# MeteoSwiss/flexpart

Hardware: AMD Instinct MI355X
Metric: particle-steps/sec (whole node) + achieved HBM GB/s, 1e8 particles (higher is better)
Workload: dtype f64

## Files before the change

### flexpart_amd/_lib.py

```python
from __future__ import annotations

import ctypes as C
import os

HERE = os.path.dirname(os.path.abspath(__file__))
LIB_PATH = os.environ.get("FPX_LIBRARY") or os.path.join(HERE, "csrc", "libflexpart_amd.so")

FPX_MAXSPEC = 5
DEAD = -999999999
RNG_TABLE_SEQ, RNG_TABLE_COUNTER, RNG_PHILOX = 0, 1, 2


class FpxConfig(C.Structure):
    _fields_ = [
        ("struct_bytes", C.c_int32), ("device", C.c_int32),
        ("compute_real_bytes", C.c_int32), ("host_real_bytes", C.c_int32),
        ("max_particles", C.c_int64),
        ("nx", C.c_int32), ("ny", C.c_int32), ("nz", C.c_int32), ("nmixz", C.c_int32),
        ("nxmax", C.c_int32), ("nymax", C.c_int32), ("nzmax", C.c_int32),
        ("dx", C.c_double), ("dy", C.c_double), ("xlon0", C.c_double), ("ylat0", C.c_double),
        ("xglobal", C.c_int32), ("nglobal", C.c_int32), ("sglobal", C.c_int32),
        ("switchnorthg", C.c_double), ("switchsouthg", C.c_double),
        ("northpolemap", C.c_double * 9), ("southpolemap", C.c_double * 9),
        ("ldirect", C.c_int32), ("lsynctime", C.c_int32), ("method", C.c_int32),
# ... 131 lines not shown
class FpxStepStats(C.Structure):
    _fields_ = [(n, C.c_int64) for n in
                ("n_due", "n_initialized", "n_left_domain", "n_min_mass", "n_max_age",
                 "nan_count", "nan_count2", "n_bad_position")] + [("kernel_ms", C.c_double)]


ALLREDUCE_FN = C.CFUNCTYPE(C.c_int, C.c_void_p, C.c_void_p, C.c_void_p, C.c_int64, C.c_int32)

SYMBOLS = [
    "fpx_create", "fpx_destroy", "fpx_last_error", "fpx_abi_version", "fpx_polar_maps", "fpx_set_height",
    "fpx_upload_fields", "fpx_set_windtime", "fpx_rng_fill_table", "fpx_rng_set_table",
    "fpx_rng_get_table", "fpx_upload_particles", "fpx_download_particles", "fpx_set_numpart", "fpx_set_release_points", "fpx_set_release_heights", "fpx_release_init", "fpx_releaseparticles", "fpx_split_particles", "fpx_redist_plan", "fpx_redist_bytes", "fpx_redist_pack", "fpx_redist_unpack",
    "fpx_step", "fpx_step_async", "fpx_sync", "fpx_counters", "fpx_kernel_time", "fpx_kernel_times", "fpx_sort_particles",
    "fpx_seed_particles", "fpx_stream", "fpx_outgrid_init", "fpx_set_output_times", "fpx_conccalc",
    "fpx_get_grids", "fpx_comm_unique_id", "fpx_comm_init", "fpx_comm_init_host", "fpx_count_particles", "fpx_lane_stats", "fpx_set_option", "fpx_get_info", "fpx_wet_init", "fpx_upload_wet_fields",
    "fpx_wetdepo", "fpx_get_wetgrid", "fpx_nests_init", "fpx_upload_nest_fields", "fpx_math_probe",
    "fpx_outgrid_nest_init", "fpx_get_grids_nest", "fpx_receptors_init", "fpx_get_receptors", "fpx_upload_wet_nest_fields",
    "fpx_verttransform_ecmwf", "fpx_verttransform_nest", "fpx_verttransform_time", "fpx_calcpar", "fpx_calcpar_time", "fpx_upload_diag_fields", "fpx_partoutput", "fpx_partoutput_time", "fpx_readpartpositions", "fpx_concoutput",
    "fpx_checkpoint_write", "fpx_checkpoint_read",
    "fpx_conv_init", "fpx_upload_conv_fields", "fpx_convmix", "fpx_convmix_time", "fpx_get_cbaseflux", "fpx_set_cbaseflux",
    "fpx_upload_conv_nest_fields", "fpx_get_cbaseflux_nest", "fpx_set_cbaseflux_nest", "fpx_upload_diag_nest_fields",
]

_lib = None


def load():
    global _lib
    if _lib is not None:
        return _lib
    if not os.path.exists(LIB_PATH):
        raise ImportError(
            f"{LIB_PATH} not found: the HIP extension is not built "
            "(run `python -c 'import __graft_entry__ as g; g.build()'`). "
            "flexpart_amd has no CPU fallback.")
    lib = C.CDLL(LIB_PATH)
    vp = C.c_void_p
    lib.fpx_last_error.restype = C.c_char_p
    lib.fpx_stream.restype = vp
    lib.fpx_stream.argtypes = [vp]
    lib.fpx_math_probe.argtypes = [C.c_int32, vp, vp, C.c_int64]
    lib.fpx_upload_wet_nest_fields.argtypes = [vp, C.c_int32, C.c_int32, C.POINTER(FpxWetFields), C.c_int32]
    lib.fpx_outgrid_nest_init.argtypes = [vp, C.POINTER(FpxOutgridNest)]
    lib.fpx_get_grids_nest.argtypes = [vp, vp, vp, vp, C.c_int32, C.c_int32]
    lib.fpx_receptors_init.argtypes = [vp, C.c_int32, vp, vp, vp]
    lib.fpx_get_receptors.argtypes = [vp, vp, C.c_int32, C.c_int32, C.c_int32]
    lib.fpx_create.argtypes = [C.POINTER(vp), C.POINTER(FpxConfig)]
    lib.fpx_destroy.argtypes = [vp]
    lib.fpx_polar_maps.argtypes = [C.c_int32, C.c_double, C.POINTER(C.c_double), C.POINTER(C.c_double)]
    lib.fpx_set_height.argtypes = [vp, vp, C.c_int32]
    lib.fpx_upload_fields.argtypes = [vp, C.c_int32, C.POINTER(FpxFields)]
    lib.fpx_verttransform_ecmwf.argtypes = [vp, C.c_int32, C.POINTER(FpxModelLevels), C.POINTER(FpxFields), C.POINTER(FpxFieldsOut)]
    lib.fpx_verttransform_nest.argtypes = [vp, C.c_int32, C.c_int32, C.POINTER(FpxModelLevels), C.POINTER(FpxFields), C.POINTER(FpxFieldsOut)]
    lib.fpx_verttransform_time.argtypes = [vp, C.POINTER(C.c_double)]
    lib.fpx_calcpar.argtypes = [vp, C.c_int32, C.POINTER(FpxCalcparIn), C.POINTER(FpxCalcparOut)]
    lib.fpx_calcpar_time.argtypes = [vp, C.POINTER(C.c_double)]
# ... 75 lines not shown
```

### flexpart_amd/csrc/fpx_device.hpp

```cpp
#pragma once
#include "fpx_tu.hpp"
#include <hip/hip_runtime.h>
#include <stdint.h>

namespace fpx {
FPX_TU_OPEN

#define K(x) ((R)(x))
#define FPX_DEV __device__ __forceinline__
#define FPX_HD __host__ __device__ __forceinline__

constexpr int kMaxSpec = 5;
constexpr int kMaxNests = 4;
constexpr int kDead = -999999999;

FPX_HD float m_exp(float x) { return expf(x); }
FPX_HD double m_exp(double x) { return exp(x); }
FPX_HD float m_log(float x) { return logf(x); }
FPX_HD double m_log(double x) { return log(x); }
FPX_HD float m_sqrt(float x) { return sqrtf(x); }
FPX_HD double m_sqrt(double x) { return sqrt(x); }
FPX_HD float m_fma(float a, float b, float c) { return fmaf(a, b, c); }
FPX_HD double m_fma(double a, double b, double c) { return fma(a, b, c); }
FPX_HD float m_sin(float x) { return sinf(x); }
// ... 630 lines not shown
  const double r = m_rcbrt(x);
  const double d = ((1.0 / 3.0) - .33333) * M.logabs(x);
  return (x * (r * r)) * (1.0 - d * (1.0 - d * (0.5 - d * 0.16666666666666666)));
}
template <typename MS>
FPX_DEV float m_pow13(float x, const MS &) { return m_powr(x, 0.33333f); }

template <typename R, typename MS>
FPX_DEV R tlw_unstable(const Turb<R> &T, R z, const MS &M) {
  if (z < m_abs(T.ol)) return K(0.1) * z * m_rcp(T.sigw * (K(0.55) - K(0.38) * m_abs(z * m_rcp(T.ol))));
  if (T.zeta < K(0.1)) return K(0.59) * z * m_rcp(T.sigw);
  return K(0.15) * T.h * m_rcp(T.sigw) * (K(1.) - M.expt(K(-5) * T.zeta));
}

template <typename R, typename MS>
FPX_DEV void sigw_unstable(Turb<R> &T, const MS &M) {
  R z23, zm13;
  zeta_powers(T.zeta, M, z23, zm13);
  T.sigw = m_sqrtp(K(1.2) * (T.wst * T.wst) * (K(1.) - K(.9) * T.zeta) * z23 + (K(1.8) - K(1.4) * T.zeta) * (T.ust * T.ust)) + K(1.e-2);
  T.dsigwdz = K(0.5) * m_rcp(T.sigw * T.h) * (K(-1.4) * (T.ust * T.ust) + (T.wst * T.wst) * (K(0.8) * zm13 - K(1.8) * z23));
}

template <typename R, typename MS = PlainMath>
FPX_DEV void hanna(Turb<R> &T, R z, const MS &M = MS()) {
  if (T.h / m_abs(T.ol) < K(1.)) {
    T.ust = m_max(K(1.e-4), T.ust);
    R corr = z * m_rcp(T.ust);
    T.sigu = K(1.e-2) + K(2.0) * T.ust * M.expt(K(-3.e-4) * corr);
    T.sigw = K(1.3) * T.ust * M.expt(K(-2.e-4) * corr);
    T.dsigwdz = K(-2.e-4) * T.sigw;
    T.sigw = T.sigw + K(1.e-2);
    T.sigv = T.sigw;
    T.tlu = K(0.5) * z * m_rcp(T.sigw * (K(1.) + K(1.5e-3) * corr));
    T.tlv = T.tlu;
    T.tlw = T.tlu;
  } else if (T.ol < K(0.)) {
// ... 2 lines not shown
    sigw_unstable(T, M);
    T.tlu = K(0.15) * T.h * m_rcp(T.sigu);
    T.tlv = T.tlu;
    T.tlw = tlw_unstable(T, z, M);
  } else {
    T.sigu = K(1.e-2) + K(2.) * T.ust * (K(1.) - T.zeta);
    T.sigv = K(1.e-2) + K(1.3) * T.ust * (K(1.) - T.zeta);
    T.sigw = T.sigv;
    T.dsigwdz = K(-1.3) * T.ust * m_rcp(T.h);
    T.tlu = K(0.15) * T.h * m_rcp(T.sigu) * m_sqrtp(T.zeta);
    T.tlv = K(0.467) * T.tlu;
    T.tlw = K(0.1) * T.h * m_rcp(T.sigw) * m_pow08(T.zeta);
  }
  T.tlu = m_max(K(10.), T.tlu);
  T.tlv = m_max(K(10.), T.tlv);
  T.tlw = m_max(K(30.), T.tlw);
  if (T.dsigwdz == K(0.)) T.dsigwdz = K(1.e-10);
}

template <typename R>
FPX_DEV void hanna1(Turb<R> &T, R z) {
  if (T.h / m_abs(T.ol) < K(1.)) {
    T.ust = m_max(K(1.e-4), T.ust);
    T.sigu = K(2.0) * T.ust * m_exp(K(-3.e-4) * z / T.ust);
    T.sigu = m_max(T.sigu, K(1.e-5));
    T.sigv = K(1.3) * T.ust * m_exp(K(-2.e-4) * z / T.ust);
    T.sigv = m_max(T.sigv, K(1.e-5));
    T.sigw = T.sigv;
    T.dsigw2dz = K(-6.76e-4) * T.ust * m_exp(K(-4.e-4) * z / T.ust);
    T.tlu = K(0.5) * z / T.sigw / (K(1.) + K(1.5e-3) * z / T.ust);
// ... 36 lines not shown
    T.dsigw2dz = K(3.38) * T.ust * T.ust * (T.zeta - K(1.)) / T.h;
    T.tlu = K(0.15) * T.h / T.sigu * m_sqrt(T.zeta);
    T.tlv = K(0.467) * T.tlu;
    T.tlw = K(0.1) * T.h / T.sigw * m_powr(T.zeta, K(0.8));
  }
  T.tlu = m_max(K(10.), T.tlu);
  T.tlv = m_max(K(10.), T.tlv);
  T.tlw = m_max(K(30.), T.tlw);
}

enum StashSlot {
  S_U, S_V, S_W,
  S_DDX, S_DDY,
  S_DX, S_DY, S_DAW, S_DCW,
  S_UP, S_VP,
  S_UST, S_WST, S_OL, S_TRANS,
  S_RHOAUX,
  S_NPASS,
  S_COUNT_LEAN,
  S_TDEP = S_COUNT_LEAN,
  S_SETCELL,
  S_SET_NUM, S_SET_DQ6, S_SET_V0,
  S_COUNT_AERO64,
  S_RT_TAG = S_COUNT_AERO64, S_RT_RHO1, S_RT_TT1, S_RT_RHO2, S_RT_TT2,
  S_COUNT
};
template <typename R> constexpr int stash_slots(bool lean, bool susp = true) { return lean ? (susp ? (int)S_COUNT_LEAN : (int)S_NPASS) : (sizeof(R) == 8 ? (int)S_COUNT_AERO64 : (int)S_COUNT); }
constexpr int kStashStride = 256;
template <typename R>
struct Stash {
  typedef __attribute__((address_space(3))) volatile R *lds_ptr;
  lds_ptr p;
  lds_tab_ptr tab;
  FPX_DEV double logabs(double x) const { return m_log_abs(x, tab); }
  FPX_DEV double expt(double x) const { return m_exp_tab(x, tab + kLdsExpTabAt); }
  FPX_DEV float logabs(float x) const { return m_logp(x); }
  FPX_DEV float expt(float x) const { return m_expp(x); }
  FPX_DEV R get(int k) const { return p[k * kStashStride]; }
  FPX_DEV void put(int k, R v) const { p[k * kStashStride] = v; }
  FPX_DEV void add(int k, R v) const { p[k * kStashStride] = p[k * kStashStride] + v; }
};

template <typename R>
struct HsInv {
  R ih, iaux;
  int regime;
};
template <typename R>
FPX_DEV HsInv<R> hanna_short_prepare(Turb<R> &T) {
  HsInv<R> I;
  I.ih = m_rcp(T.h);
  if (T.h / m_abs(T.ol) < K(1.)) {
    I.regime = 0;
    T.ust = m_max(K(1.e-4), T.ust);
    I.iaux = m_rcp(T.ust);
  } else if (T.ol < K(0.)) {
    I.regime = 1;
    I.iaux = m_rcp(T.ol);
  } else {
    I.regime = 2;
    I.iaux = K(0.);
  }
  return I;
}

template <typename R, typename ST>
FPX_DEV void hanna_short(Turb<R> &T, R z, const HsInv<R> &I, const ST &S) {
  if (I.regime == 0) {
    const R corr = z * I.iaux;
    T.sigw = K(1.3) * S.expt(K(-2.e-4) * corr);
    T.dsigwdz = K(-2.e-4) * T.sigw;
    T.sigw = T.sigw * S.get(S_UST) + K(1.e-2);
    const R qn = K(1.) + K(1.5e-3) * corr;
    const R in2 = m_rcp(T.sigw * qn);
    T.isigw = in2 * qn;
    T.tlw = K(0.5) * z * in2;
  } else if (I.regime == 1) {
    R z23, zm13;
    zeta_powers(T.zeta, S, z23, zm13);
    const R ust = S.get(S_UST), wst = S.get(S_WST);
    const R ust2 = ust * ust, wst2 = wst * wst;
    T.sigw = m_sqrtp(K(1.2) * wst2 * (K(1.) - K(.9) * T.zeta) * z23 + (K(1.8) - K(1.4) * T.zeta) * ust2) + K(1.e-2);
    const bool low = z < m_abs(S.get(S_OL));
    const R q = low ? K(0.55) - K(0.38) * m_abs(z * I.iaux) : K(1.);
    const R i2 = m_rcp(T.sigw * q);
    const R isig = i2 * q;
    T.isigw = isig;
    T.dsigwdz = K(0.5) * isig * I.ih * (K(-1.4) * ust2 + wst2 * (K(0.8) * zm13 - K(1.8) * z23));
    if (low) T.tlw = K(0.1) * z * i2;
    else if (T.zeta < K(0.1)) T.tlw = K(0.59) * z * isig;
    else T.tlw = K(0.15) * T.h * isig * (K(1.) - S.expt(K(-5) * T.zeta));
  } else {
    const R ust = S.get(S_UST);
    T.sigw = K(1.e-2) + K(1.3) * ust * (K(1.) - T.zeta);
    T.dsigwdz = K(-1.3) * ust * I.ih;
    T.isigw = m_rcp(T.sigw);
// ... 10 lines not shown

template <typename R>
FPX_DEV R cuberoot(R x) { return m_sign(m_pow(m_abs(x), K(0.333333333)), x); }

template <typename R>
FPX_DEV R cbl_transition(R h, R ol) {
  R transition = K(1.);
  if (-h / ol < K(15)) transition = m_sin(((-h / ol + K(10.)) / K(10.)) * FPX_PI_PAR) / K(2.) + K(0.5);
  return transition;
}

template <typename R, typename ST>
FPX_DEV void cbl(const ST &S, int ldirect, R wp, R zp, R wt , R ih , R rhoaux , R sigmaw, R irw , R dsigmawdz, R tlw,
                 R &ath, R &bth, int &flagrein) {
  const R usurad2 = K(0.7071067812), usurad2p = K(0.3989422804), C0 = K(3), costluar4 = K(0.66667), eps = K(0.000001);
  const R timedir = (R)ldirect;
  const R z = zp * ih;
  const R w2 = sigmaw * sigmaw;
  const R rtl = m_rsqrt(tlw);
  const R alfa = (K(2.) / C0) * w2 * (rtl * rtl);
  const R wold = timedir * wp;
  const R omz = K(1.) - z;
  const R omz05 = m_sqrtp(omz), omz15 = omz * omz05;
  const R w3 = (K(1.2) * z * omz15 + eps) * wt;
  const R dw3 = (K(1.2) * (omz15 - z * K(1.5) * omz05)) * (wt * ih);
  const R irw2 = irw * irw, irw3 = irw2 * irw;
  const R skew = w3 * irw3;
  const R dskew = irw3 * dw3 - K(3.) * skew * dsigmawdz * irw;
  R fluarw = K(0.), dfluarw = K(0.), xluarw = K(0.), dxluarw = K(0.);
  if (skew != K(0)) {
    R croot, icroot2;
    m_cuberoot_parts(m_abs(skew), croot, icroot2);
    fluarw = costluar4 * m_sign(croot, skew);
    dfluarw = costluar4 * (K(1.) / K(3.)) * icroot2 * dskew;
  }
  const R fluarw2 = fluarw * fluarw;
// ... 37 lines not shown
  const R pb = (usurad2p * isb) * eb;
  const R aperfa = da * usurad2;
  const R aperfb = db * usurad2;
  const R rx = rhoaux;
  const R apa = aluarw * pa, bpb = bluarw * pb;
  const R ptot = apa + bpb;
  const R Ta = aluarw * (dwa + wa * rx) + wa * daluarw;
  const R Tb = bluarw * (dwb + wb * rx) + wb * dbluarw;
  const R wdf = wold * dfluarw;
  const R Ua = sigmawa * (aluarw * (dsigmawa * (wold2 * isa2 + K(1.)) + wdf) + sigmawa * (daluarw + rx * aluarw));
  const R Ub = sigmawb * (bluarw * (dsigmawb * (wold2 * isb2 + K(1.)) - wdf) + sigmawb * (dbluarw + rx * bluarw));
  const R cu = usurad2 * usurad2 - K(0.5);
  R erfa, erfb;
  m_erf_e2(aperfa, ea - ea * (da2 * cu), aperfb, eb - eb * (db2 * cu), erfa, erfb);
  const R Phi = K(0.5) * (Tb * erfb - Ta * erfa) + Ua * pa + Ub * pb;
  const R Q = timedir * ((da * isa) * apa + (db * isb) * bpb);
  ath = m_rcp(ptot) * (-(C0 / K(2.)) * alfa * Q + Phi);
  bth = (sigmaw * K(1.4142135623730951)) * rtl;
}

template <typename R>
FPX_DEV void cbl_pdf(R zp, R wst, R h, R sigmaw, R ol, R &aluarw, R &sigmawa, R &sigmawb, R &wa, R &wb) {
  const R costluar4 = K(0.66667), eps = K(0.000001);
  R z = zp / h;
  R transition = cbl_transition(h, ol);
  R w2 = sigmaw * sigmaw;
  const R omz = K(1.) - z;
  R w3 = ((K(1.2) * z * (omz * m_sqrt(omz)) + eps) * (wst * wst * wst)) * transition;
  R radw2 = m_sqrt(w2);
  R skew = w3 / (w2 * radw2);
  R skew2 = skew * skew;
// ... 853 lines not shown
  const bool h1 = V.m1 != 0, h2 = V.m2 != 0;
#pragma unroll
  for (int lev = 0; lev < 2; lev++) {
    R y[5];
#pragma unroll
    for (int k = 0; k < 5; k++) {
      const R y1 = k < 3 ? (h1 ? a3[lev][1][k] : a3[lev][0][k]) : (h1 ? a2[lev][1][k - 3] : a2[lev][0][k - 3]);
      const R y2 = k < 3 ? (h2 ? a3[lev][1][k] : a3[lev][0][k]) : (h2 ? a2[lev][1][k - 3] : a2[lev][0][k - 3]);
      y[k] = (y1 * W.dt2 + y2 * W.dt1) * W.dtt;
    }
#pragma unroll
    for (int k = 0; k < 5; k++) lv[lev][k] = y[k];
  }
}

template <int T>
FPX_DEV bool sw(int runtime) { return T < 0 ? runtime != 0 : T != 0; }

template <typename R, bool DRYDEP, bool SETTLE, int TSW, int CBLF, typename RNG>
FPX_DEV int pbl_pass(const View<R> &V, const R *hgt, const RNG &G, const TimeW<R> &W, int itime, double xt, double yt,
                     R &zt, R &wp, int &ldt, short &icbt, LoopCtx<R> &A, const Stash<R> &S,
                     int &indz_last, Stats *st) {
  const R eps = V.eps;
  const R eps2 = K(1.e-9);
  const R href = K(15.);
  const R h = A.h;
  const Fld<R> F = fld_of(V, A.ngrid);
  int nrand = A.nrand;
  const bool turbswitch = sw<TSW>(V.turbswitch);
  const bool cblflag = sw<CBLF>(V.cblflag == 1);
  const bool turboff = TSW < 0 && V.turboff != 0;
  Turb<R> T;
  T.ust = S.get(S_UST); T.wst = S.get(S_WST); T.ol = S.get(S_OL); T.h = h;
  T.sigw = K(0.); T.dsigw2dz = K(0.); T.dsigwdz = K(0.);

  if (V.method == 1) {
    ldt = min(ldt, abs(V.lsynctime - A.itimec + itime));
    A.itimec = A.itimec + ldt * V.ldirect;
  } else {
    ldt = abs(V.lsynctime);
    A.itimec = itime + V.lsynctime;
  }
  const R dt = (R)ldt;
  T.zeta = zt / h;

  const int indz = find_level(hgt, V.nz, zt);
  const int indzp = indz + 1;
  indz_last = indz;
// ... 5 lines not shown
  const R dz2 = (hgt[indzp - 1] - zt) * dz;
  {
    const R u = dz1 * lv[1][0] + dz2 * lv[0][0];
    const R v = dz1 * lv[1][1] + dz2 * lv[0][1];
    S.put(S_U, u); S.put(S_V, v);
    S.put(S_W, dz1 * lv[1][2] + dz2 * lv[0][2]);
    S.add(S_DX, u * dt);
    S.add(S_DY, v * dt);
  }
  {
    const R rhoa = dz1 * lv[1][3] + dz2 * lv[0][3];
    const R rhograd = dz1 * lv[1][4] + dz2 * lv[0][4];
    S.put(S_RHOAUX, rhograd * m_rcp(rhoa));
  }

  if (turbswitch) hanna(T, zt, S); else hanna1(T, zt);
  S.put(S_UST, T.ust);
  T.isigw = m_rcp(T.sigw);

  if (RNG::kCounter) nrand = (nrand + 3) & ~3;
  if (nrand + 1 > V.maxrand) nrand = 1;
  {
    const R g1 = G.at(nrand), g2 = G.at(nrand + 1);
    const R dttlu = dt * m_rcp(T.tlu), dttlv = dt * m_rcp(T.tlv);
    R up = S.get(S_UP), vp = S.get(S_VP);
    if (dttlu < K(.5)) {
      up = (K(1.) - dttlu) * up + g1 * T.sigu * m_sqrtp(K(2.) * dttlu);
    } else {
      R ru = S.expt(-dttlu);
      up = ru * up + g1 * T.sigu * m_sqrtp(K(1.) - ru * ru);
    }
    if (dttlv < K(.5)) {
      vp = (K(1.) - dttlv) * vp + g2 * T.sigv * m_sqrtp(K(2.) * dttlv);
    } else {
      R rv = S.expt(-dttlv);
      vp = rv * vp + g2 * T.sigv * m_sqrtp(K(1.) - rv * rv);
    }
    if (turboff) { up = K(0.); vp = K(0.); }
    S.put(S_UP, up); S.put(S_VP, vp);
    S.add(S_DAW, up * dt);
    S.add(S_DCW, vp * dt);
  }
  nrand = nrand + 2;

  if (nrand + V.ifine > V.maxrand) nrand = 1;
  const R dtf = dt * V.fine;
  const R dtftlw = dtf * m_rcp(T.tlw);
  const bool cbl_on = cblflag && (-h / T.ol > K(5));
  const R sqrt_dtf = m_sqrtp(dtf);
  const HsInv<R> HI = hanna_short_prepare(T);

  FPX_LANES(st, 0);
  unsigned int flip = icbt < 0 ? 0x80000000u : 0u;
  for (int i = 1; i <= V.ifine; i++) {
    R delz;
    FPX_LANES(st, 1);
    if (turbswitch) {
      if (dtftlw < K(.5)) {
        if (cblflag) {
          if (cbl_on) {
            FPX_LANES(st, 2);
            int flagrein = 0;
            nrand = nrand + 1;
            R old_wp_buf = wp, ath, bth;
            cbl(S, V.ldirect, wp, zt, S.get(S_TRANS), HI.ih, S.get(S_RHOAUX), T.sigw, T.isigw, T.dsigwdz, T.tlw, ath, bth, flagrein);
            wp = m_flip(wp + ath * dtf + bth * G.at(nrand) * sqrt_dtf, flip);
            delz = wp * dtf;
            if (__builtin_expect(flagrein == 1, 0)) {
              re_initialize_particle(V.ldirect, G, zt, S.get(S_WST), h, T.sigw, old_wp_buf, nrand, S.get(S_OL));
              wp = old_wp_buf;
              delz = wp * dtf;
              atomicAdd(&st->nan_count, 1ull);
            }
          } else {
            FPX_LANES(st, 3);
            nrand = nrand + 1;
            R ath = -wp * m_rcp(T.tlw) + T.sigw * T.dsigwdz + wp * wp * T.isigw * T.dsigwdz + T.sigw * T.sigw * S.get(S_RHOAUX);
            R bth = T.sigw * G.at(nrand) * m_sqrtp(K(2.) * dtftlw);
            wp = m_flip(wp + ath * dtf + bth, flip);
            delz = wp * dtf;
            if (__builtin_expect(!isfinite(wp), 0)) {
              nrand = nrand + 1;
              wp = T.sigw * G.at(nrand);
              delz = wp * dtf;
              atomicAdd(&st->nan_count2, 1ull);
            }
          }
        } else {
          wp = m_flip((K(1.) - dtftlw) * wp + G.at(nrand + i) * m_sqrtp(K(2.) * dtftlw) + dtf * (T.dsigwdz + S.get(S_RHOAUX) * T.sigw), flip);
          delz = wp * T.sigw * dtf;
        }
      } else {
        FPX_LANES(st, 4);
        R rw = S.expt(-dtftlw);
        wp = m_flip(rw * wp + G.at(nrand + i) * m_sqrtp(K(1.) - rw * rw) + T.tlw * (K(1.) - rw) * (T.dsigwdz + S.get(S_RHOAUX) * T.sigw), flip);
        delz = wp * T.sigw * dtf;
      }
    } else {
      R rw = m_expp(-dtftlw);
      wp = m_flip(rw * wp + G.at(nrand + i) * m_sqrtp(K(1.) - rw * rw) * T.sigw + T.tlw * (K(1.) - rw) * (T.dsigw2dz + S.get(S_RHOAUX) * (T.sigw * T.sigw)), flip);
      delz = wp * dtf;
    }

    if (turboff) { wp = K(0.); delz = K(0.); }

    if (__builtin_expect(m_abs(delz) > h, 0)) delz = m_fmod(delz, h);
    {
      const bool below = delz < -zt, above = !below && delz > (h - zt);
      flip = (below || above) ? 0x80000000u : 0u;
      const R base = zt + delz;
      const R lift = above ? K(2.) * h : K(0.);
      zt = m_flip(base, flip) + lift;
    }
    if (i != V.ifine) {
      T.zeta = zt * HI.ih;
#ifdef FPX_LANE_STATS
      if (HI.regime == 0) FPX_LANES(st, 5); else if (HI.regime == 1) FPX_LANES(st, 6); else FPX_LANES(st, 7);
#endif
      hanna_short(T, zt, HI, S);
    }
  }
// ... 613 lines not shown
```

### flexpart_amd/csrc/fpx_engine.hip

```cpp
#include <hip/hip_runtime.h>
#include <cstddef>
#include <cstring>
#include <rccl/rccl.h>
#include <rocprim/device/device_radix_sort.hpp>
#include <rocprim/device/device_scan.hpp>
#include <rocprim/device/device_select.hpp>
#include <rocprim/iterator/counting_iterator.hpp>
#include <algorithm>
#include <cmath>
#include <cstdio>
#include <cstring>
#include <string>
#include <vector>

#include "../../include/flexpart_amd.h"
#include "fpx_tu.hpp"
#include "fpx_device.hpp"
#include "fpx_verttransform.hpp"
#include "fpx_calcpar.hpp"
#include "fpx_convect.hpp"
#include "fpx_rng_host.hpp"

namespace fpx {

// ... 401 lines not shown
  }
  P.xt[s] = ps.xt; P.yt[s] = ps.yt; P.zt[s] = ps.zt;
  if (TURB) { P.up[s] = ps.up; P.vp[s] = ps.vp; P.cbt[s] = ps.icbt; }
  P.wp[s] = ps.wp;
  P.us[s] = ps.usigold; P.vs[s] = ps.vsigold; P.ws[s] = ps.wsigold;
  P.idt[s] = ps.ldt; P.itra1[s] = itra1;
}

enum { PBL_FRESH = 3 };
template <typename R>
struct alignas(16 * sizeof(R)) PblRecord {
  R v[13];
  int i[3];
};
static_assert(sizeof(PblRecord<double>) == 128 && sizeof(PblRecord<float>) == 64, "one cache line / half a line per record");
__device__ __forceinline__ int pbl_pack(int state, int icbt, int indz, int ngrid, int elapsed) {
  return state | (icbt < 0 ? 4 : 0) | (indz << 3) | ((ngrid + 2) << 12) | (elapsed << 15);
}
__device__ __forceinline__ int pbl_state(int pk) { return pk & 3; }
__device__ __forceinline__ int pbl_icbt(int pk) { return (pk & 4) ? -1 : 1; }
__device__ __forceinline__ int pbl_indz(int pk) { return (pk >> 3) & 511; }
__device__ __forceinline__ int pbl_ngrid(int pk) { return ((pk >> 12) & 7) - 2; }
__device__ __forceinline__ int pbl_elapsed(int pk) { return (pk >> 15) & 65535; }
static_assert(kMaxNz <= 512 && kMaxNests + 2 <= 7, "pbl_pack field widths");
template <typename R>
struct PblRec {
  PblRecord<R> *rec;
  R *tdep;
};

// ... 25 lines not shown
    atomicAdd(&st->n_init, 1ull);
  }

  AdvCtx<R> A;
  const TimeW<R> W = time_weights(V, itime);
  const bool in_pbl = adv_begin<R, MOTHER, true>(V, ps.xt, ps.yt, ps.zt, itime, advance_start_index(V, S, G, pid), A);
  if (V.lsettling) A.nsp = settling_species(V, P.npoint[s]);
  if (in_pbl) {
    if (is_new) {
      P.up[s] = ps.up; P.vp[s] = ps.vp; P.wp[s] = ps.wp;
      P.us[s] = ps.usigold; P.vs[s] = ps.vsigold; P.ws[s] = ps.wsigold;
      P.idt[s] = ps.ldt; P.cbt[s] = ps.icbt;
    }
    PblCtx<R> B;
    pbl_begin(V, ps.xt, ps.yt, W, A, B);
    {
      PblRecord<R> &r = Q.rec[s];
      r.v[8] = B.ust; r.v[9] = B.wst; r.v[10] = B.ol; r.v[11] = B.transition;
      r.v[12] = A.h;
      r.i[0] = A.nrand; r.i[2] = pbl_pack(PBL_FRESH, 1, 0, A.ngrid, 0);
    }
    unsigned char cls;
    if (V.cblflag == 1 && V.turbswitch && (-A.h / B.ol > (R)5)) cls = 1;
    else if (A.h / m_abs(B.ol) < (R)1) cls = 3;
    else if (B.ol < (R)0) cls = 2;
    else cls = 4;
    unsigned char bucket = 0;
    if (V.pbl_cost_buckets) {
      const int idt = is_new ? ps.ldt : P.idt[s];
      const int est = abs(V.lsynctime) / max(idt, 1);
      if (V.pbl_cost_buckets == 1) bucket = est >= 128 ? 3 : est >= 64 ? 2 : est >= 32 ? 1 : 0;
      else if (V.pbl_cost_buckets == 2) bucket = est >= 64 ? 1 : 0;
      else bucket = est >= 256 ? 7 : est >= 128 ? 6 : est >= 96 ? 5 : est >= 64 ? 4 : est >= 48 ? 3 : est >= 32 ? 2 : est >= 16 ? 1 : 0;
    }
    pbl_flag[s] = (unsigned char)((cls - 1) * 8 + (7 - bucket));
    return;
  }
  R usig, vsig, wsig;
  pbl_flag[s] = kKeyDone;
  auto late = [&]() {
// ... 707 lines not shown
          t_x = wall_clock64();
#endif
        }
      }
      if (cur < end) {
        const unsigned int rank = __popcll(need & ((1ull << lane) - 1ull));
        const unsigned int my = cur + rank;
        const unsigned int s_new = (unsigned int)__builtin_amdgcn_ds_bpermute((int)(min(my - cbase, 63u) << 2), (int)ahead);
        if (!have && my < end) {
          FPX_LANES(st, 8);
          s = s_new;
          const PblRecord<R> *rp = Q.rec + s;
          const double l_xt = P.xt[s], l_yt = P.yt[s];
          const unsigned int l_pid = P.pid[s];
          const int r_nrand = rp->i[0], r_ldt = SUSP ? rp->i[1] : 0, r_pk = rp->i[2];
          const R r_ust = rp->v[8], r_wst = rp->v[9], r_ol = rp->v[10], r_trans = rp->v[11], r_h = rp->v[12];
          R l_zt = P.zt[s], l_wp = P.wp[s], l_up = P.up[s], l_vp = P.vp[s];
          int l_idt = P.idt[s];
          short l_cbt = P.cbt[s];
          const R c_dx = SUSP ? rp->v[0] : (R)0, c_dy = SUSP ? rp->v[1] : (R)0, c_daw = SUSP ? rp->v[2] : (R)0, c_dcw = SUSP ? rp->v[3] : (R)0;
          const R c_zt = SUSP ? rp->v[4] : (R)0, c_up = SUSP ? rp->v[5] : (R)0, c_vp = SUSP ? rp->v[6] : (R)0, c_wp = SUSP ? rp->v[7] : (R)0;
          int l_npoint = 0;
          if (!LEAN && V.lsettling) l_npoint = P.npoint[s];
          R c_tdep = (R)0;
          if (SUSP && !LEAN && V.drydep) c_tdep = Q.tdep[s];
          __builtin_amdgcn_sched_barrier(0);
          const bool resumed = SUSP && pbl_state(r_pk) == PBL_CONTINUE;
          xt = l_xt; yt = l_yt; pid = l_pid;
          zt = resumed ? c_zt : l_zt; wp = resumed ? c_wp : l_wp;
          ldt = resumed ? r_ldt : l_idt;
          icbt = resumed ? (short)pbl_icbt(r_pk) : l_cbt;
// ... 5 lines not shown
            A.nsp = 0;
            if (!LEAN && V.lsettling) {
              const int nsp = settling_species(V, l_npoint);
              const SettleSpec<R> sp = settle_spec(V, nsp);
              S.put(S_SET_NUM, spec_row(V, nsp).density > (R)0 ? sp.num : (R)0);
              S.put(S_SET_DQ6, sp.dq6); S.put(S_SET_V0, sp.vset);
              S.put(S_SETCELL, (R)settling_column(V, (R)xt, (R)yt));
              if (sizeof(R) == 4) S.put(S_RT_TAG, (R)0);
            }
            S.put(S_DDX, ddx); S.put(S_DDY, ddy);
          }
          S.put(S_DX, resumed ? c_dx : (R)0); S.put(S_DY, resumed ? c_dy : (R)0);
          S.put(S_DAW, resumed ? c_daw : (R)0); S.put(S_DCW, resumed ? c_dcw : (R)0);
          S.put(S_W, (R)0);
          S.put(S_UP, resumed ? c_up : l_up); S.put(S_VP, resumed ? c_vp : l_vp);
          S.put(S_UST, r_ust); S.put(S_WST, r_wst); S.put(S_OL, r_ol);
          S.put(S_TRANS, (r_wst * r_wst * r_wst) * r_trans);
          if (SUSP) S.put(S_NPASS, (R)0);
          if (!LEAN && V.drydep) S.put(S_TDEP, resumed ? c_tdep : (R)0);
          have = true;
        }
        cur = min(cur + (unsigned int)__popcll(need), end);
      }
    }
    if (!__any(have)) {
      if (out_of_chunks) break;
      continue;
    }
    bool over_budget = false;
    if (have) {
      Rng<R, RNGM> G;
      make_rng(V, pid, step, G);
      int indz = 1;
      const int rc = pbl_pass<R, !LEAN, !LEAN, TSW, CBLF>(V, hgt, G, W, itime, xt, yt, zt, wp, ldt, icbt, A, S, indz, st);
      R npass = (R)0;
      if (SUSP) { npass = S.get(S_NPASS) + (R)1; S.put(S_NPASS, npass); }
      if (rc != PBL_CONTINUE) {
        FPX_LANES(st, 9);
        write_record(rc, indz);
        have = false;
      } else over_budget = SUSP && npass >= cap_r;
    }
    if (SUSP && cap_passes > 0) suspend(over_budget);
  }
#ifdef FPX_LANE_STATS
  if (lane == 0) {
    const unsigned long long t_e = wall_clock64();
    atomicAdd(&st->lanes[11][0], 1ull);
    atomicAdd(&st->lanes[11][1], t_x - t_s);
// ... 13 lines not shown
  switch (fn) {
    case 0: r = m_expp(v); break;
    case 1: r = m_logp(v); break;
    case 2: r = m_sqrtp(v); break;
    case 3: r = m_rcp(v); break;
    case 4: r = m_rsqrt(v); break;
    case 5: m_cuberoot_parts(v, c, ic2); r = c; break;
    case 7: r = m_erf_e(v, m_expp(-(v * v))); break;
    case 8: r = m_pow08(v); break;
    case 9: r = m_exp_tab(v, &kExpTab[0]); break;
    case 10: r = m_log_abs(v); break;
    case 11: r = m_rcbrt(v); break;
    default: m_cuberoot_parts(v, c, ic2); r = ic2; break;
  }
  y[i] = r;
}

template <typename R, bool DRYDEP, bool POLAR, bool NEST, bool CAPCHECK>
__device__ __forceinline__ void finish_body(const View<R> &V, const GridP<R> &Gp, Parts<R> &P, unsigned int s, const PblRecord<R> &rec, R tdep,
                                            int itime, unsigned int step, Stats *st, const R *hgt, DryDep<R> *dry) {
  constexpr bool MOTHER = !POLAR && !NEST;
  const int pk = rec.i[2];
  PState<R> ps;
  ps.xt = P.xt[s]; ps.yt = P.yt[s]; ps.zt = rec.v[4];
  ps.up = rec.v[5]; ps.vp = rec.v[6]; ps.wp = rec.v[7];
  ps.usigold = P.us[s]; ps.vsigold = P.vs[s]; ps.wsigold = P.ws[s];
  ps.ldt = rec.i[1]; ps.icbt = (short)pbl_icbt(pk);
  Rng<R> G;
  make_rng(V, P.pid[s], step, G);
  const TimeW<R> W = time_weights(V, itime);
// ... 3775 lines not shown
  if (fn < 0 || fn > 11 || !x || !y || n < 0) return FPX_ERR_ARG;
  if (n == 0) return FPX_OK;
  double *dx = nullptr, *dy = nullptr;
  if (hipMalloc(&dx, n * sizeof(double)) != hipSuccess) return FPX_ERR_NOMEM;
  if (hipMalloc(&dy, n * sizeof(double)) != hipSuccess) { (void)hipFree(dx); return FPX_ERR_NOMEM; }
  hipError_t e = hipMemcpy(dx, x, n * sizeof(double), hipMemcpyHostToDevice);
  if (e == hipSuccess) {
    fpx::k_math_probe<<<(unsigned)((n + fpx::kBlock - 1) / fpx::kBlock), fpx::kBlock>>>(fn, dx, dy, n);
    e = hipGetLastError();
  }
  if (e == hipSuccess) e = hipMemcpy(y, dy, n * sizeof(double), hipMemcpyDeviceToHost);
  (void)hipFree(dx); (void)hipFree(dy);
  return e == hipSuccess ? FPX_OK : FPX_ERR_DEVICE;
}

}
#endif
```

### include/flexpart_amd.h

```cpp
#ifndef FLEXPART_AMD_H
#define FLEXPART_AMD_H

#include <stdint.h>

#ifdef __cplusplus
extern "C" {
#endif

#define FPX_MAXSPEC 5
#define FPX_MAXNESTS 4
#define FPX_DEAD (-999999999)

typedef struct fpx_engine *fpx_handle;

typedef enum {
  FPX_OK = 0,
  FPX_ERR_ARG = -1,
  FPX_ERR_DEVICE = -2,
  FPX_ERR_STATE = -3,
  FPX_ERR_NOMEM = -4,
  FPX_ERR_UNSUPPORTED = -5
} fpx_status;

typedef enum { FPX_RNG_TABLE_SEQ = 0, FPX_RNG_TABLE_COUNTER = 1, FPX_RNG_PHILOX = 2 } fpx_rng_mode;
// ... 266 lines not shown

typedef struct {
  int32_t struct_bytes;
  int32_t numxgridn, numygridn;
  double dxoutn, dyoutn, xoutshiftn, youtshiftn;
  int32_t reserved[4];
} fpx_outgrid_nest;
int fpx_outgrid_nest_init(fpx_handle h, const fpx_outgrid_nest *g);
int fpx_get_grids_nest(fpx_handle h, void *griduncn, void *drygriduncn, void *wetgriduncn, int32_t allreduce, int32_t clear);
int fpx_receptors_init(fpx_handle h, int32_t numreceptor, const void *xreceptor, const void *yreceptor, const void *receptorarea);
int fpx_get_receptors(fpx_handle h, void *creceptor, int32_t ld, int32_t allreduce, int32_t clear);

void *fpx_stream(fpx_handle h);

int fpx_math_probe(int32_t fn, const double *x, double *y, int64_t n);
int fpx_lane_stats(fpx_handle h, uint64_t *out, int32_t n, int32_t reset);

int fpx_set_option(fpx_handle h, const char *name, const char *value);
int fpx_get_info(fpx_handle h, const char *name, int64_t *value);

#ifdef __cplusplus
}
#endif
#endif
```

Baseline: 372.8 million.

## Hoist per-step Hanna turbulence invariants out of the PBL inner loop

Adds step_invariants, which computes regime flags, reciprocal of ust or ol, the unstable sigu and the inverse Lagrangian time for u once per particle step. These values are stored in the PBL record or the LDS stash and consumed by a new hanna overload, so the per-pass pow13, reciprocal and branch work is not recomputed. The stash holds wst squared instead of wst, and raw wst is reloaded from the record only on cold paths. It also replaces timedir multiplies with sign flips, adds asm barriers to steer scheduling, and adds a probe kernel for checking equivalence. The cost is extra stash slots and record writes, which may raise LDS use and register pressure.

```diff
diff --git a/flexpart_amd/_lib.py b/flexpart_amd/_lib.py
--- a/flexpart_amd/_lib.py
+++ b/flexpart_amd/_lib.py
@@ -169,7 +169,7 @@
     "fpx_step", "fpx_step_async", "fpx_sync", "fpx_counters", "fpx_kernel_time", "fpx_kernel_times", "fpx_sort_particles",
     "fpx_seed_particles", "fpx_stream", "fpx_outgrid_init", "fpx_set_output_times", "fpx_conccalc",
     "fpx_get_grids", "fpx_comm_unique_id", "fpx_comm_init", "fpx_comm_init_host", "fpx_count_particles", "fpx_lane_stats", "fpx_set_option", "fpx_get_info", "fpx_wet_init", "fpx_upload_wet_fields",
-    "fpx_wetdepo", "fpx_get_wetgrid", "fpx_nests_init", "fpx_upload_nest_fields", "fpx_math_probe",
+    "fpx_wetdepo", "fpx_get_wetgrid", "fpx_nests_init", "fpx_upload_nest_fields", "fpx_math_probe", "fpx_hanna_probe",
     "fpx_outgrid_nest_init", "fpx_get_grids_nest", "fpx_receptors_init", "fpx_get_receptors", "fpx_upload_wet_nest_fields",
     "fpx_verttransform_ecmwf", "fpx_verttransform_nest", "fpx_verttransform_time", "fpx_calcpar", "fpx_calcpar_time", "fpx_upload_diag_fields", "fpx_partoutput", "fpx_partoutput_time", "fpx_readpartpositions", "fpx_concoutput",
     "fpx_checkpoint_write", "fpx_checkpoint_read",
@@ -195,6 +195,7 @@
     lib.fpx_stream.restype = vp
     lib.fpx_stream.argtypes = [vp]
     lib.fpx_math_probe.argtypes = [C.c_int32, vp, vp, C.c_int64]
+    lib.fpx_hanna_probe.argtypes = [vp, vp, C.c_int64]
     lib.fpx_upload_wet_nest_fields.argtypes = [vp, C.c_int32, C.c_int32, C.POINTER(FpxWetFields), C.c_int32]
     lib.fpx_outgrid_nest_init.argtypes = [vp, C.POINTER(FpxOutgridNest)]
     lib.fpx_get_grids_nest.argtypes = [vp, vp, vp, vp, C.c_int32, C.c_int32]
diff --git a/flexpart_amd/csrc/fpx_device.hpp b/flexpart_amd/csrc/fpx_device.hpp
--- a/flexpart_amd/csrc/fpx_device.hpp
+++ b/flexpart_amd/csrc/fpx_device.hpp
@@ -668,12 +668,14 @@
 }
 
 template <typename R, typename MS>
-FPX_DEV void sigw_unstable(Turb<R> &T, const MS &M) {
+FPX_DEV void sigw_unstable(Turb<R> &T, R ust2, R wst2, const MS &M) {
   R z23, zm13;
   zeta_powers(T.zeta, M, z23, zm13);
-  T.sigw = m_sqrtp(K(1.2) * (T.wst * T.wst) * (K(1.) - K(.9) * T.zeta) * z23 + (K(1.8) - K(1.4) * T.zeta) * (T.ust * T.ust)) + K(1.e-2);
-  T.dsigwdz = K(0.5) * m_rcp(T.sigw * T.h) * (K(-1.4) * (T.ust * T.ust) + (T.wst * T.wst) * (K(0.8) * zm13 - K(1.8) * z23));
-}
+  T.sigw = m_sqrtp(K(1.2) * wst2 * (K(1.) - K(.9) * T.zeta) * z23 + (K(1.8) - K(1.4) * T.zeta) * ust2) + K(1.e-2);
+  T.dsigwdz = K(0.5) * m_rcp(T.sigw * T.h) * (K(-1.4) * ust2 + wst2 * (K(0.8) * zm13 - K(1.8) * z23));
+}
+template <typename R, typename MS>
+FPX_DEV void sigw_unstable(Turb<R> &T, const MS &M) { sigw_unstable(T, T.ust * T.ust, T.wst * T.wst, M); }
 
 template <typename R, typename MS = PlainMath>
 FPX_DEV void hanna(Turb<R> &T, R z, const MS &M = MS()) {
@@ -706,6 +708,75 @@
   }
   T.tlu = m_max(K(10.), T.tlu);
   T.tlv = m_max(K(10.), T.tlv);
+  T.tlw = m_max(K(30.), T.tlw);
+  if (T.dsigwdz == K(0.)) T.dsigwdz = K(1.e-10);
+}
+
+enum { INV_REGIME = 3, INV_DEEP = 4 };
+template <typename R>
+struct StepInv {
+  R ust;
+  R iaux;
+  R sigu, itlu;
+  int flags;
+};
+template <typename R, typename MS>
+FPX_DEV StepInv<R> step_invariants(R h, R ol, R ust, R wst, const MS &M) {
+  StepInv<R> I;
+  I.ust = ust; I.sigu = K(0.); I.itlu = K(0.);
+  if (h / m_abs(ol) < K(1.)) {
+    I.flags = 0;
+    I.ust = m_max(K(1.e-4), ust);
+    I.iaux = m_rcp(I.ust);
+  } else if (ol < K(0.)) {
+    I.flags = 1;
+    I.iaux = m_rcp(ol);
+    I.sigu = K(1.e-2) + ust * m_pow13(K(12) - K(0.5) * h * I.iaux, M);
+    I.itlu = m_rcp(m_max(K(10.), K(0.15) * h * m_rcp(I.sigu)));
+  } else {
+    I.flags = 2;
+    I.iaux = K(0.);
+  }
+  if (-h / ol > K(5)) I.flags |= INV_DEEP;
+  return I;
+}
+
+template <typename R, typename INV, typename MS>
+FPX_DEV void hanna(Turb<R> &T, R z, const INV &I, const MS &M, R &itlu, R &itlv) {
+  const int regime = I.regime();
+  if (regime == 0) {
+    R corr = z * I.get_iaux();
+    T.sigu = K(1.e-2) + K(2.0) * T.ust * M.expt(K(-3.e-4) * corr);
+    T.sigw = K(1.3) * T.ust * M.expt(K(-2.e-4) * corr);
+    T.dsigwdz = K(-2.e-4) * T.sigw;
+    T.sigw = T.sigw + K(1.e-2);
+    T.sigv = T.sigw;
+    T.tlu = K(0.5) * z * m_rcp(T.sigw * (K(1.) + K(1.5e-3) * corr));
+    T.tlv = T.tlu;
+    T.tlw = T.tlu;
+  } else if (regime == 1) {
+    T.sigu = I.get_sigu();
+    T.sigv = T.sigu;
+    sigw_unstable(T, T.ust * T.ust, I.get_wst2(), M);
+    if (z < m_abs(T.ol)) T.tlw = K(0.1) * z * m_rcp(T.sigw * (K(0.55) - K(0.38) * m_abs(z * I.get_iaux())));
+    else if (T.zeta < K(0.1)) T.tlw = K(0.59) * z * m_rcp(T.sigw);
+    else T.tlw = K(0.15) * T.h * m_rcp(T.sigw) * (K(1.) - M.expt(K(-5) * T.zeta));
+  } else {
+    T.sigu = K(1.e-2) + K(2.) * T.ust * (K(1.) - T.zeta);
+    T.sigv = K(1.e-2) + K(1.3) * T.ust * (K(1.) - T.zeta);
+    T.sigw = T.sigv;
+    T.dsigwdz = K(-1.3) * T.ust * m_rcp(T.h);
+    T.tlu = K(0.15) * T.h * m_rcp(T.sigu) * m_sqrtp(T.zeta);
+    T.tlv = K(0.467) * T.tlu;
+    T.tlw = K(0.1) * T.h * m_rcp(T.sigw) * m_pow08(T.zeta);
+  }
+  if (regime == 1) {
+    itlu = I.get_itlu(); itlv = itlu;
+  } else {
+    T.tlu = m_max(K(10.), T.tlu);
+    T.tlv = m_max(K(10.), T.tlv);
+    itlu = m_rcp(T.tlu); itlv = m_rcp(T.tlv);
+  }
   T.tlw = m_max(K(30.), T.tlw);
   if (T.dsigwdz == K(0.)) T.dsigwdz = K(1.e-10);
 }
@@ -772,7 +843,8 @@
   S_DDX, S_DDY,
   S_DX, S_DY, S_DAW, S_DCW,
   S_UP, S_VP,
-  S_UST, S_WST, S_OL, S_TRANS,
+  S_UST, S_WST2, S_OL, S_TRANS,
+  S_IAUX, S_SIGU, S_ITLU,
   S_RHOAUX,
   S_NPASS,
   S_COUNT_LEAN,
@@ -800,27 +872,25 @@
 };
 
 template <typename R>
+FPX_DEV R inv_pack_itlu(const StepInv<R> &I) { return m_flip(I.itlu, (I.flags & INV_DEEP) ? 0x80000000u : 0u); }
+FPX_DEV bool m_signbit(double x) { return __double2hiint(x) < 0; }
+FPX_DEV bool m_signbit(float x) { return (int)__float_as_uint(x) < 0; }
+template <typename R>
+struct StashInv {
+  const Stash<R> &S;
+  FPX_DEV int regime() const { const R iaux = S.get(S_IAUX); return iaux > K(0.) ? 0 : iaux < K(0.) ? 1 : 2; }
+  FPX_DEV bool deep() const { return m_signbit(S.get(S_ITLU)); }
+  FPX_DEV R get_iaux() const { return S.get(S_IAUX); }
+  FPX_DEV R get_sigu() const { return S.get(S_SIGU); }
+  FPX_DEV R get_itlu() const { return m_abs(S.get(S_ITLU)); }
+  FPX_DEV R get_wst2() const { return S.get(S_WST2); }
+};
+
+template <typename R>
 struct HsInv {
   R ih, iaux;
   int regime;
 };
-template <typename R>
-FPX_DEV HsInv<R> hanna_short_prepare(Turb<R> &T) {
-  HsInv<R> I;
-  I.ih = m_rcp(T.h);
-  if (T.h / m_abs(T.ol) < K(1.)) {
-    I.regime = 0;
-    T.ust = m_max(K(1.e-4), T.ust);
-    I.iaux = m_rcp(T.ust);
-  } else if (T.ol < K(0.)) {
-    I.regime = 1;
-    I.iaux = m_rcp(T.ol);
-  } else {
-    I.regime = 2;
-    I.iaux = K(0.);
-  }
-  return I;
-}
 
 template <typename R, typename ST>
 FPX_DEV void hanna_short(Turb<R> &T, R z, const HsInv<R> &I, const ST &S) {
@@ -836,8 +906,8 @@
   } else if (I.regime == 1) {
     R z23, zm13;
     zeta_powers(T.zeta, S, z23, zm13);
-    const R ust = S.get(S_UST), wst = S.get(S_WST);
-    const R ust2 = ust * ust, wst2 = wst * wst;
+    const R ust = S.get(S_UST);
+    const R ust2 = ust * ust, wst2 = S.get(S_WST2);
     T.sigw = m_sqrtp(K(1.2) * wst2 * (K(1.) - K(.9) * T.zeta) * z23 + (K(1.8) - K(1.4) * T.zeta) * ust2) + K(1.e-2);
     const bool low = z < m_abs(S.get(S_OL));
     const R q = low ? K(0.55) - K(0.38) * m_abs(z * I.iaux) : K(1.);
@@ -878,12 +948,12 @@
 FPX_DEV void cbl(const ST &S, int ldirect, R wp, R zp, R wt , R ih , R rhoaux , R sigmaw, R irw , R dsigmawdz, R tlw,
                  R &ath, R &bth, int &flagrein) {
   const R usurad2 = K(0.7071067812), usurad2p = K(0.3989422804), C0 = K(3), costluar4 = K(0.66667), eps = K(0.000001);
-  const R timedir = (R)ldirect;
+  const unsigned int tdir = ldirect < 0 ? 0x80000000u : 0u;
   const R z = zp * ih;
   const R w2 = sigmaw * sigmaw;
   const R rtl = m_rsqrt(tlw);
   const R alfa = (K(2.) / C0) * w2 * (rtl * rtl);
-  const R wold = timedir * wp;
+  const R wold = m_flip(wp, tdir);
   const R omz = K(1.) - z;
   const R omz05 = m_sqrtp(omz), omz15 = omz * omz05;
   const R w3 = (K(1.2) * z * omz15 + eps) * wt;
@@ -951,7 +1021,7 @@
   R erfa, erfb;
   m_erf_e2(aperfa, ea - ea * (da2 * cu), aperfb, eb - eb * (db2 * cu), erfa, erfb);
   const R Phi = K(0.5) * (Tb * erfb - Ta * erfa) + Ua * pa + Ub * pb;
-  const R Q = timedir * ((da * isa) * apa + (db * isb) * bpb);
+  const R Q = m_flip((da * isa) * apa + (db * isb) * bpb, tdir);
   ath = m_rcp(ptot) * (-(C0 / K(2.)) * alfa * Q + Phi);
   bth = (sigmaw * K(1.4142135623730951)) * rtl;
 }
@@ -1835,13 +1905,25 @@
   }
 }
 
+constexpr int kRecStride = 16, kRecWst = 9;
+template <typename R>
+struct RecCold {
+  const R *v0;
+  unsigned int slot;
+  FPX_DEV R wst() const {
+    unsigned int s = slot;
+    asm volatile("" : "+v"(s));
+    return v0[(size_t)s * kRecStride + kRecWst];
+  }
+};
+
 template <int T>
 FPX_DEV bool sw(int runtime) { return T < 0 ? runtime != 0 : T != 0; }
 
 template <typename R, bool DRYDEP, bool SETTLE, int TSW, int CBLF, typename RNG>
 FPX_DEV int pbl_pass(const View<R> &V, const R *hgt, const RNG &G, const TimeW<R> &W, int itime, double xt, double yt,
                      R &zt, R &wp, int &ldt, short &icbt, LoopCtx<R> &A, const Stash<R> &S,
-                     int &indz_last, Stats *st) {
+                     int &indz_last, Stats *st, const RecCold<R> &RC) {
   const R eps = V.eps;
   const R eps2 = K(1.e-9);
   const R href = K(15.);
@@ -1852,7 +1934,7 @@
   const bool cblflag = sw<CBLF>(V.cblflag == 1);
   const bool turboff = TSW < 0 && V.turboff != 0;
   Turb<R> T;
-  T.ust = S.get(S_UST); T.wst = S.get(S_WST); T.ol = S.get(S_OL); T.h = h;
+  T.h = h;
   T.sigw = K(0.); T.dsigw2dz = K(0.); T.dsigwdz = K(0.);
 
   if (V.method == 1) {
@@ -1888,15 +1970,19 @@
     S.put(S_RHOAUX, rhograd * m_rcp(rhoa));
   }
 
-  if (turbswitch) hanna(T, zt, S); else hanna1(T, zt);
-  S.put(S_UST, T.ust);
+  const StashInv<R> SI{S};
+  T.ust = S.get(S_UST); T.ol = S.get(S_OL);
+  if (!turbswitch) T.wst = RC.wst();
+  R itlu, itlv;
+  if (turbswitch) hanna(T, zt, SI, S, itlu, itlv);
+  else { hanna1(T, zt); S.put(S_UST, T.ust); itlu = m_rcp(T.tlu); itlv = m_rcp(T.tlv); }
   T.isigw = m_rcp(T.sigw);
 
   if (RNG::kCounter) nrand = (nrand + 3) & ~3;
   if (nrand + 1 > V.maxrand) nrand = 1;
   {
     const R g1 = G.at(nrand), g2 = G.at(nrand + 1);
-    const R dttlu = dt * m_rcp(T.tlu), dttlv = dt * m_rcp(T.tlv);
+    const R dttlu = dt * itlu, dttlv = dt * itlv;
     R up = S.get(S_UP), vp = S.get(S_VP);
     if (dttlu < K(.5)) {
       up = (K(1.) - dttlu) * up + g1 * T.sigu * m_sqrtp(K(2.) * dttlu);
@@ -1920,9 +2006,9 @@
   if (nrand + V.ifine > V.maxrand) nrand = 1;
   const R dtf = dt * V.fine;
   const R dtftlw = dtf * m_rcp(T.tlw);
-  const bool cbl_on = cblflag && (-h / T.ol > K(5));
+  const bool cbl_on = cblflag && SI.deep();
   const R sqrt_dtf = m_sqrtp(dtf);
-  const HsInv<R> HI = hanna_short_prepare(T);
+  const HsInv<R> HI{m_rcp(h), SI.get_iaux(), SI.regime()};
 
   FPX_LANES(st, 0);
   unsigned int flip = icbt < 0 ? 0x80000000u : 0u;
@@ -1941,7 +2027,8 @@
             wp = m_flip(wp + ath * dtf + bth * G.at(nrand) * sqrt_dtf, flip);
             delz = wp * dtf;
             if (__builtin_expect(flagrein == 1, 0)) {
-              re_initialize_particle(V.ldirect, G, zt, S.get(S_WST), h, T.sigw, old_wp_buf, nrand, S.get(S_OL));
+              const R wst = RC.wst();
+              re_initialize_particle(V.ldirect, G, zt, wst, h, T.sigw, old_wp_buf, nrand, S.get(S_OL));
               wp = old_wp_buf;
               delz = wp * dtf;
               atomicAdd(&st->nan_count, 1ull);
@@ -1966,7 +2053,9 @@
         }
       } else {
         FPX_LANES(st, 4);
-        R rw = S.expt(-dtftlw);
+        R xw = dtftlw;
+        asm volatile("" : "+v"(xw));
+        R rw = S.expt(-xw);
         wp = m_flip(rw * wp + G.at(nrand + i) * m_sqrtp(K(1.) - rw * rw) + T.tlw * (K(1.) - rw) * (T.dsigwdz + S.get(S_RHOAUX) * T.sigw), flip);
         delz = wp * T.sigw * dtf;
       }
@@ -1978,7 +2067,7 @@
 
     if (turboff) { wp = K(0.); delz = K(0.); }
 
-    if (__builtin_expect(m_abs(delz) > h, 0)) delz = m_fmod(delz, h);
+    if (__builtin_expect(m_abs(delz) > h, 0)) { R hh = h; asm volatile("" : "+v"(hh)); delz = m_fmod(delz, hh); }
     {
       const bool below = delz < -zt, above = !below && delz > (h - zt);
       flip = (below || above) ? 0x80000000u : 0u;
diff --git a/flexpart_amd/csrc/fpx_engine.hip b/flexpart_amd/csrc/fpx_engine.hip
--- a/flexpart_amd/csrc/fpx_engine.hip
+++ b/flexpart_amd/csrc/fpx_engine.hip
@@ -439,6 +439,8 @@
   int i[3];
 };
 static_assert(sizeof(PblRecord<double>) == 128 && sizeof(PblRecord<float>) == 64, "one cache line / half a line per record");
+static_assert(sizeof(PblRecord<double>) == kRecStride * sizeof(double) && sizeof(PblRecord<float>) == kRecStride * sizeof(float) &&
+              offsetof(PblRecord<double>, v) == 0 && offsetof(PblRecord<float>, v) == 0 && kRecWst < 13, "RecCold (fpx_device.hpp) indexes the records by these");
 __device__ __forceinline__ int pbl_pack(int state, int icbt, int indz, int ngrid, int elapsed) {
   return state | (icbt < 0 ? 4 : 0) | (indz << 3) | ((ngrid + 2) << 12) | (elapsed << 15);
 }
@@ -494,16 +496,18 @@
     }
     PblCtx<R> B;
     pbl_begin(V, ps.xt, ps.yt, W, A, B);
+    const StepInv<R> I = step_invariants(A.h, B.ol, B.ust, B.wst, PlainMath());
     {
       PblRecord<R> &r = Q.rec[s];
-      r.v[8] = B.ust; r.v[9] = B.wst; r.v[10] = B.ol; r.v[11] = B.transition;
+      r.v[8] = I.ust; r.v[kRecWst] = B.wst; r.v[10] = B.ol; r.v[11] = B.transition;
       r.v[12] = A.h;
+      r.v[0] = I.iaux; r.v[1] = I.sigu; r.v[2] = inv_pack_itlu(I);
       r.i[0] = A.nrand; r.i[2] = pbl_pack(PBL_FRESH, 1, 0, A.ngrid, 0);
     }
     unsigned char cls;
-    if (V.cblflag == 1 && V.turbswitch && (-A.h / B.ol > (R)5)) cls = 1;
-    else if (A.h / m_abs(B.ol) < (R)1) cls = 3;
-    else if (B.ol < (R)0) cls = 2;
+    if (V.cblflag == 1 && V.turbswitch && (I.flags & INV_DEEP)) cls = 1;
+    else if ((I.flags & INV_REGIME) == 0) cls = 3;
+    else if ((I.flags & INV_REGIME) == 1) cls = 2;
     else cls = 4;
     unsigned char bucket = 0;
     if (V.pbl_cost_buckets) {
@@ -1241,7 +1245,8 @@
           const double l_xt = P.xt[s], l_yt = P.yt[s];
           const unsigned int l_pid = P.pid[s];
           const int r_nrand = rp->i[0], r_ldt = SUSP ? rp->i[1] : 0, r_pk = rp->i[2];
-          const R r_ust = rp->v[8], r_wst = rp->v[9], r_ol = rp->v[10], r_trans = rp->v[11], r_h = rp->v[12];
+          const R r_ust = rp->v[8], r_wst = rp->v[kRecWst], r_ol = rp->v[10], r_trans = rp->v[11], r_h = rp->v[12];
+          const R r_iaux = SUSP ? (R)0 : rp->v[0], r_sigu = SUSP ? (R)0 : rp->v[1], r_itlu = SUSP ? (R)0 : rp->v[2];
           R l_zt = P.zt[s], l_wp = P.wp[s], l_up = P.up[s], l_vp = P.vp[s];
           int l_idt = P.idt[s];
           short l_cbt = P.cbt[s];
@@ -1277,10 +1282,18 @@
           S.put(S_DAW, resumed ? c_daw : (R)0); S.put(S_DCW, resumed ? c_dcw : (R)0);
           S.put(S_W, (R)0);
           S.put(S_UP, resumed ? c_up : l_up); S.put(S_VP, resumed ? c_vp : l_vp);
-          S.put(S_UST, r_ust); S.put(S_WST, r_wst); S.put(S_OL, r_ol);
+          S.put(S_WST2, r_wst * r_wst);
+          S.put(S_OL, r_ol);
           S.put(S_TRANS, (r_wst * r_wst * r_wst) * r_trans);
           if (SUSP) S.put(S_NPASS, (R)0);
           if (!LEAN && V.drydep) S.put(S_TDEP, resumed ? c_tdep : (R)0);
+          if (SUSP) {
+            __builtin_amdgcn_sched_barrier(0);
+            const StepInv<R> I = step_invariants(r_h, r_ol, r_ust, r_wst, S);
+            S.put(S_UST, I.ust); S.put(S_IAUX, I.iaux); S.put(S_SIGU, I.sigu); S.put(S_ITLU, inv_pack_itlu(I));
+          } else {
+            S.put(S_UST, r_ust); S.put(S_IAUX, r_iaux); S.put(S_SIGU, r_sigu); S.put(S_ITLU, r_itlu);
+          }
           have = true;
         }
         cur = min(cur + (unsigned int)__popcll(need), end);
@@ -1295,7 +1308,7 @@
       Rng<R, RNGM> G;
       make_rng(V, pid, step, G);
       int indz = 1;
-      const int rc = pbl_pass<R, !LEAN, !LEAN, TSW, CBLF>(V, hgt, G, W, itime, xt, yt, zt, wp, ldt, icbt, A, S, indz, st);
+      const int rc = pbl_pass<R, !LEAN, !LEAN, TSW, CBLF>(V, hgt, G, W, itime, xt, yt, zt, wp, ldt, icbt, A, S, indz, st, RecCold<R>{Q.rec[0].v, s});
       R npass = (R)0;
       if (SUSP) { npass = S.get(S_NPASS) + (R)1; S.put(S_NPASS, npass); }
       if (rc != PBL_CONTINUE) {
@@ -1339,6 +1352,37 @@
     default: m_cuberoot_parts(v, c, ic2); r = ic2; break;
   }
   y[i] = r;
+}
+
+__global__ void __launch_bounds__(kBlock) k_hanna_probe(int which, const double *__restrict__ in, double *__restrict__ out, long long n) {
+  __shared__ double slots[(S_ITLU + 1) * kStashStride];
+  __shared__ double lds_tab[kLdsTabDoubles];
+  for (int k = threadIdx.x; k < kLdsTabDoubles; k += blockDim.x) lds_tab[k] = k < kLdsExpTabAt ? kLogTab[k >> 1][k & 1] : kExpTab[k - kLdsExpTabAt];
+  __syncthreads();
+  const long long i = (long long)blockIdx.x * blockDim.x + threadIdx.x;
+  if (i >= n) return;
+  const double h = in[5 * i], ol = in[5 * i + 1], ust = in[5 * i + 2], wst = in[5 * i + 3], z = in[5 * i + 4];
+  double *o = out + 10 * i;
+  Turb<double> T;
+  T.ol = ol; T.h = h; T.zeta = z / h; T.sigw = 0.; T.dsigwdz = 0.;
+  if (which == 0) {
+    const Stash<double> S{(Stash<double>::lds_ptr)(slots + threadIdx.x), (lds_tab_ptr)lds_tab};
+    const StepInv<double> I = step_invariants(h, ol, ust, wst, PlainMath());
+    S.put(S_UST, I.ust); S.put(S_OL, ol); S.put(S_WST2, wst * wst);
+    S.put(S_IAUX, I.iaux); S.put(S_SIGU, I.sigu); S.put(S_ITLU, inv_pack_itlu(I));
+    const StashInv<double> SI{S};
+    T.ust = S.get(S_UST);
+    double itlu, itlv;
+    hanna(T, z, SI, S, itlu, itlv);
+    o[0] = T.sigu; o[1] = T.sigv; o[2] = T.sigw; o[3] = T.dsigwdz; o[4] = itlu; o[5] = itlv; o[6] = T.tlw;
+    o[7] = T.ust; o[8] = (double)SI.regime(); o[9] = SI.deep() ? 1. : 0.;
+  } else {
+    T.ust = ust; T.wst = wst;
+    const bool deep = -h / T.ol > 5.;
+    hanna(T, z, Stash<double>{nullptr, (lds_tab_ptr)lds_tab});
+    o[0] = T.sigu; o[1] = T.sigv; o[2] = T.sigw; o[3] = T.dsigwdz; o[4] = m_rcp(T.tlu); o[5] = m_rcp(T.tlv); o[6] = T.tlw;
+    o[7] = T.ust; o[8] = h / m_abs(ol) < 1. ? 0. : ol < 0. ? 1. : 2.; o[9] = deep ? 1. : 0.;
+  }
 }
 
 template <typename R, bool DRYDEP, bool POLAR, bool NEST, bool CAPCHECK>
@@ -5144,5 +5188,21 @@
   return e == hipSuccess ? FPX_OK : FPX_ERR_DEVICE;
 }
 
+int fpx_hanna_probe(const double *in, double *out, int64_t n) {
+  if (!in || !out || n < 0) return FPX_ERR_ARG;
+  if (n == 0) return FPX_OK;
+  double *dx = nullptr, *dy = nullptr;
+  if (hipMalloc(&dx, 5 * n * sizeof(double)) != hipSuccess) return FPX_ERR_NOMEM;
+  if (hipMalloc(&dy, 10 * n * sizeof(double)) != hipSuccess) { (void)hipFree(dx); return FPX_ERR_NOMEM; }
+  hipError_t e = hipMemcpy(dx, in, 5 * n * sizeof(double), hipMemcpyHostToDevice);
+  for (int which = 0; which < 2 && e == hipSuccess; which++) {
+    fpx::k_hanna_probe<<<(unsigned)((n + fpx::kBlock - 1) / fpx::kBlock), fpx::kBlock>>>(which, dx, dy, n);
+    e = hipGetLastError();
+    if (e == hipSuccess) e = hipMemcpy(out + 10 * n * which, dy, 10 * n * sizeof(double), hipMemcpyDeviceToHost);
+  }
+  (void)hipFree(dx); (void)hipFree(dy);
+  return e == hipSuccess ? FPX_OK : FPX_ERR_DEVICE;
+}
+
 }
 #endif
diff --git a/include/flexpart_amd.h b/include/flexpart_amd.h
--- a/include/flexpart_amd.h
+++ b/include/flexpart_amd.h
@@ -304,6 +304,7 @@
 void *fpx_stream(fpx_handle h);
 
 int fpx_math_probe(int32_t fn, const double *x, double *y, int64_t n);
+int fpx_hanna_probe(const double *in, double *out, int64_t n);
 int fpx_lane_stats(fpx_handle h, uint64_t *out, int32_t n, int32_t reset);
 
 int fpx_set_option(fpx_handle h, const char *name, const char *value);
```

After: 382.2 million, median of 6. 2.5% higher.
